# mratsim/constantine

Hardware: AMD Instinct MI355X
Metric: MSM points/sec, BLS12-381 G1, 2^20 random pairs; pipelined throughput, 2 MSMs in flight, inputs resident in HBM (higher is better)
Workload: dtype u32; 1 GPU; bls12_381_g1 MSM, 2^20 (scalar,point) pairs per GPU, inputs resident in HBM, 2 MSMs in flight (BASELINE.json configs[1]); pairs_per_gpu=1048576, total_pairs=1048576, ranks=1, scalar_bits=255, window_bits=16, windows=16, entries_per_lane=131, seed=1592590338

## Files before the change

constantine_amd/csrc/hip_backend.h:

```cpp
#pragma once
#include <hip/hip_runtime.h>

#include "generators.h"
#include "hip_errors.h"
#include "msm_pipeline.h"

namespace ctt {

#define HIP_CHECK(expr)                                                                              \
  do {                                                                                               \
    hipError_t e_ = (expr);                                                                          \
    if (e_ != hipSuccess)                                                                            \
      ::ctt::hip_failed(#expr, hipGetErrorString(e_), e_ == hipErrorOutOfMemory, __FILE__, __LINE__); \
  } while (0)

template <class Fr>
__global__ void k_fr_from_mont(const uint32_t* in, uint32_t* out, uint32_t n) {
  fr_from_mont_body<Fr>(in, out, n, blockIdx.x * blockDim.x + threadIdx.x);
}

static constexpr int ACCUM_BLOCK = 64;

static constexpr int EC_BLOCK = 64;

// ... 16 lines not shown
    const Affine<F> p = in[j];
    r.v.a.x = FD::from_sat(p.x);
    r.v.a.y = FD::from_sat(p.y);
    r.w[gather_flag_offset<FD>() / 4u] = p.is_inf() ? 1u : 0u;
#pragma unroll
    for (uint32_t i = 0; i < CH; i++) cv_lds[t * CH + (i ^ (t & (CH - 1u)))] = r.q[i];
  }
  __syncthreads();
  const uint32_t cnt = (n - j0 < (uint32_t)CONVERT_BLOCK ? n - j0 : (uint32_t)CONVERT_BLOCK) * CH;
  uint4* dst = reinterpret_cast<uint4*>((char*)out + (uint64_t)j0 * STRIDE);
  for (uint32_t i = t; i < cnt; i += CONVERT_BLOCK) {
    const uint32_t rec = i / CH, ch = i & (CH - 1u);
    dst[i] = cv_lds[rec * CH + (ch ^ (rec & (CH - 1u)))];
  }
}

#ifndef CTT_ACCUM_WAVES
#define CTT_ACCUM_WAVES 2
#endif
template <class F>
struct GatherLds {
  static constexpr uint32_t NCH = gather_chunks<F>();
  static_assert(F::UNSAT, "records in the converted layout only");
  uint4 (*stage)[ACCUM_BLOCK];
  __device__ void request(const char* rec) {
    asm volatile("s_waitcnt lgkmcnt(0)" ::: "memory");
#pragma unroll
    for (uint32_t j = 0; j < NCH; j++)
      __builtin_amdgcn_global_load_lds((const __attribute__((address_space(1))) void*)(rec + 16u * j),
                                       (__attribute__((address_space(3))) void*)&stage[j][0], 16, 0, 0);
  }
  __device__ void collect(Affine<F>& pt, bool& qinf) {
    asm volatile("s_waitcnt vmcnt(0)" ::: "memory");
    union {
      uint4 q[NCH];
      uint32_t w[NCH * 4u];
    } r;
#pragma unroll
    for (uint32_t j = 0; j < NCH; j++) r.q[j] = stage[j][threadIdx.x];
    __builtin_memcpy(&pt, r.w, sizeof(Affine<F>));
    qinf = r.w[gather_flag_offset<F>() / 4u] != 0u;
  }
};
template <class F, bool INTO = false>
__global__ void __launch_bounds__(ACCUM_BLOCK, (sizeof(XYZZ<F>) > 256 ? 1 : CTT_ACCUM_WAVES)) k_accum(AccumArgs<F> a) {
#if defined(CTT_G2_PHASE_NOPS) && CTT_G2_PHASE_NOPS > 0
  if constexpr (IsFp2<F>::value && F::UNSAT) {
#pragma unroll
    for (int i = 0; i < CTT_G2_PHASE_NOPS; i++) asm volatile("s_nop 0");
  }
#endif
  if constexpr (F::UNSAT && !IsFp2<F>::value) {
    __shared__ uint4 stage[GatherLds<F>::NCH][ACCUM_BLOCK];
    GatherLds<F> gq{stage};
    accum_body<F, GatherLds<F>, INTO>(a, blockIdx.y, blockIdx.x * blockDim.x + threadIdx.x, gq);
  } else {
    accum_body<F, INTO>(a, blockIdx.y, blockIdx.x * blockDim.x + threadIdx.x);
  }
}
template <class F>
__global__ void __launch_bounds__(EC_BLOCK) k_merge_tail(MergeArgs<F> a) {
  merge_tail_body<F>(a, blockIdx.y, blockIdx.x * blockDim.x + threadIdx.x);
}
template <class F>
__global__ void __launch_bounds__(EC_BLOCK) k_merge_step(MergeArgs<F> a, uint32_t d) {
  merge_step_body<F>(a, blockIdx.y, blockIdx.x * blockDim.x + threadIdx.x, d);
}
template <class F>
__global__ void __launch_bounds__(EC_BLOCK) k_merge_final(MergeArgs<F> a) {
  if (merge_chain_bound<F>(a) <= 1) return;
  merge_final_body<F>(a, blockIdx.y, blockIdx.x * blockDim.x + threadIdx.x);
}
template <class F>
__global__ void __launch_bounds__(EC_BLOCK) k_merge_tail_queue(MergeArgs<F> a) {
  uint32_t item = 0;
  const bool more = merge_tail_queue_body<F>(a, blockIdx.y, blockIdx.x * blockDim.x + threadIdx.x, &item);
  const uint64_t mask = __ballot(more);
  if (mask == 0) return;
  uint32_t base = 0;
  const uint32_t lane = threadIdx.x & 63u;
  if (lane == (uint32_t)(__ffsll((long long)mask) - 1)) base = atomicAdd(a.qcount, (uint32_t)__popcll(mask));
  base = __shfl(base, __ffsll((long long)mask) - 1, 64);
  if (more) a.queue[base + (uint32_t)__popcll(mask & ((1ull << lane) - 1ull))] = item;
}
template <class F>
__global__ void __launch_bounds__(EC_BLOCK) k_merge_queue(MergeArgs<F> a, uint32_t lmax) {
  merge_queue_body<F>(a, blockIdx.x * blockDim.x + threadIdx.x, lmax);
}
template <class F>
__global__ void __launch_bounds__(EC_BLOCK) k_pyr(PyrArgs<F> a, uint32_t ntasks) {
  const uint32_t t = blockIdx.x * blockDim.x + threadIdx.x;
  if (t < ntasks) pyr_body<F>(a, blockIdx.y, t);
}
// ... 180 lines not shown
    if (role == 0) {
      const XYZZ<F> x = *s1;
      *d1 = x;
      if (d2) *d2 = x;
    }
    return;
  }
  xyzz_add_quad<F>(s1, s2, d1, d2, role);
}
static constexpr int RED_BLOCK = 256;
template <class F>
__global__ void __launch_bounds__(RED_BLOCK) k_merge_finish(MergeArgs<F> a, uint32_t first_d) {
  merge_finish_body<F>(a, blockIdx.x, first_d, threadIdx.x, blockDim.x, []() { __syncthreads(); });
}
template <class F>
__global__ void __launch_bounds__(EC_BLOCK) k_merge_queue_quad(MergeArgs<F> a, uint32_t lmax) {
  const uint32_t lane = blockIdx.x * blockDim.x + threadIdx.x;
  const uint32_t qi = lane >> 2;
  const int role = (int)(lane & 3u);
  if (qi >= *a.qcount) return;
  const uint32_t slot = a.queue[qi];
  const uint32_t w = slot / a.G, s = slot - w * a.G;
  const uint32_t b = a.hkey[slot];
  const uint32_t* bs = a.bucket_start + (uint64_t)w * (a.B + 1);
  const uint32_t len = chain_last(bs, a.K, b) - s + 1;
  if (len > lmax) return;
  XYZZ<F> acc = a.heads[slot];
  for (uint32_t i = 1; i < len; i++) {
    const XYZZ<F> h = a.heads[slot + i];
    xyzz_add_quad_reg<F>(acc, h, role);
  }
  if (role == 0) a.buckets[(uint64_t)w * a.B + b] = acc;
}
template <class F>
__global__ void __launch_bounds__(RED_BLOCK) k_merge_long(MergeArgs<F> a, uint32_t lmax) {
  merge_long_body<F>(a, blockIdx.x, lmax, threadIdx.x, blockDim.x, []() { __syncthreads(); });
}
template <class F>
__global__ void __launch_bounds__(EC_BLOCK) k_merge_step_quad(MergeArgs<F> a, uint32_t d) {
  const uint32_t lane = blockIdx.x * blockDim.x + threadIdx.x;
  const uint32_t g = lane >> 2;
  if (!merge_step_active<F>(a, blockIdx.y, g, d)) return;
  XYZZ<F>* h = a.heads + (uint64_t)blockIdx.y * a.G + g;
  xyzz_add_quad<F>(h, h + d, h, (XYZZ<F>*)nullptr, (int)(lane & 3u));
}
template <class C>
__global__ void __launch_bounds__(EC_BLOCK) k_gen_points(uint64_t seed, uint64_t first, uint32_t n, Affine<typename C::F>* out) {
  Affine<typename C::F> G = generator<C>();
// ... 291 lines not shown
  }

  static dim3 grid1(uint32_t n, int block) { return dim3((n + block - 1) / block); }
  static dim3 grid2(uint32_t n, int block, uint32_t W) { return dim3((n + block - 1) / block, W); }

  template <class Fr>
  void launch_fr_from_mont(const uint32_t* in, uint32_t* out, uint32_t n) {
    hipLaunchKernelGGL(k_fr_from_mont<Fr>, grid1(n, 256), dim3(256), 0, front(), in, out, n);
    HIP_CHECK(hipGetLastError());
  }
  template <class F, class FD>
  void launch_convert(const Affine<F>* in, void* out, uint32_t n) {
    hipLaunchKernelGGL((k_convert_points<F, FD>), grid1(n, CONVERT_BLOCK), dim3(CONVERT_BLOCK),
                       (size_t)CONVERT_BLOCK * gather_stride<FD>(), front(), in, out, n);
    HIP_CHECK(hipGetLastError());
  }
  template <class F>
  void launch_table_next(const Affine<F>* prev, Affine<F>* next, uint32_t n, int c) {
    hipLaunchKernelGGL(k_table_next<F>, grid1(n, EC_BLOCK), dim3(EC_BLOCK), 0, stream, prev, next, n, c);
    HIP_CHECK(hipGetLastError());
  }
  void sync() { HIP_CHECK(hipStreamSynchronize(stream)); }
  void launch_digits_sort(const SortArgs& a);
  template <class F>
  void launch_accum(const AccumArgs<F>& a, uint32_t W, bool into = false) {
    if (into) launch_accum_into<F>(stream, a, W);
    else hipLaunchKernelGGL((k_accum<F, false>), grid2(a.G, ACCUM_BLOCK, W), dim3(ACCUM_BLOCK), 0, stream, a);
    HIP_CHECK(hipGetLastError());
  }
  template <class F>
  void launch_merge_tail(const MergeArgs<F>& a, uint32_t W) {
    hipLaunchKernelGGL(k_merge_tail<F>, grid2(a.G, EC_BLOCK, W), dim3(EC_BLOCK), 0, cur(), a);
    HIP_CHECK(hipGetLastError());
  }
  template <class F>
  void launch_merge_step(const MergeArgs<F>& a, uint32_t W, uint32_t d) {
    if ((uint64_t)a.G * W * 4u <= 1048576u) {
      hipLaunchKernelGGL(k_merge_step_quad<F>, grid2(a.G * 4u, EC_BLOCK, W), dim3(EC_BLOCK), 0, cur(), a, d);
      HIP_CHECK(hipGetLastError());
      return;
    }
    hipLaunchKernelGGL(k_merge_step<F>, grid2(a.G, EC_BLOCK, W), dim3(EC_BLOCK), 0, cur(), a, d);
    HIP_CHECK(hipGetLastError());
  }
  template <class F>
  void launch_merge_finish(const MergeArgs<F>& a, uint32_t W, uint32_t first_d) {
// ... 280 lines not shown
```

constantine_amd/csrc/msm_bodies.h:

```cpp
#pragma once
#include "ec.h"

namespace ctt {

static constexpr uint32_t DIGIT_NONE = 0xffffffffu;
static constexpr uint32_t KEY_NONE = 0xffffffffu;

struct Bls12381G1 { using F = Fp<BLS12_381_Fp>; using FD = FpU<BLS12_381_Fp_U>; using Fr = Fp<BLS12_381_Fr>; static constexpr int BITS = 255; static constexpr int ID = 0; static constexpr double ACC_NS = 0.142, RED_NS = 0.26; static constexpr int NARROW_PRIO_LOG2N = 19; static constexpr int WHOLE_TAIL_LOG2N = 0; };
struct Bls12381G2 { using F = Fp2<Fp<BLS12_381_Fp>>; using FD = Fp2<FpU<BLS12_381_Fp_U>>; using Fr = Fp<BLS12_381_Fr>; static constexpr int BITS = 255; static constexpr int ID = 1; static constexpr double ACC_NS = 0.467, RED_NS = 1.1; static constexpr int NARROW_PRIO_LOG2N = 0; static constexpr int WHOLE_TAIL_LOG2N = 0; };
struct Bn254G1 { using F = Fp<BN254_Fp>; using FD = FpU<BN254_Fp_U>; using Fr = Fp<BN254_Fr>; static constexpr int BITS = 254; static constexpr int ID = 2; static constexpr double ACC_NS = 0.0685, RED_NS = 0.12; static constexpr int NARROW_PRIO_LOG2N = 19; static constexpr int WHOLE_TAIL_LOG2N = 21; };
struct Bn254G2 { using F = Fp2<Fp<BN254_Fp>>; using FD = F; using Fr = Fp<BN254_Fr>; static constexpr int BITS = 254; static constexpr int ID = 3; static constexpr double ACC_NS = 0.5, RED_NS = 1.2; static constexpr int NARROW_PRIO_LOG2N = 0; static constexpr int WHOLE_TAIL_LOG2N = 0; };
struct PallasEc { using F = Fp<Pallas_Fp>; using FD = FpU<Pallas_Fp_U>; using Fr = Fp<Vesta_Fp>; static constexpr int BITS = 255; static constexpr int ID = 4; static constexpr double ACC_NS = 0.056, RED_NS = 0.10; static constexpr int NARROW_PRIO_LOG2N = 0; static constexpr int WHOLE_TAIL_LOG2N = 21; };
struct VestaEc { using F = Fp<Vesta_Fp>; using FD = FpU<Vesta_Fp_U>; using Fr = Fp<Pallas_Fp>; static constexpr int BITS = 255; static constexpr int ID = 5; static constexpr double ACC_NS = 0.056, RED_NS = 0.10; static constexpr int NARROW_PRIO_LOG2N = 0; static constexpr int WHOLE_TAIL_LOG2N = 21; };
struct Banderwagon { using F = Fp<Banderwagon_Fp>; using FD = F; using Fr = Fp<Banderwagon_Fr>; static constexpr int BITS = 253; static constexpr int ID = 6; static constexpr double ACC_NS = 0.12, RED_NS = 0.20; static constexpr int NARROW_PRIO_LOG2N = 0; static constexpr int WHOLE_TAIL_LOG2N = 0; };

CTT_HD uint32_t scalar_bits_at(const uint32_t* k, int pos, int nb) {
  int word = pos >> 5, sh = pos & 31;
  uint32_t lo = word < 8 ? k[word] >> sh : 0u;
  if (sh + nb > 32 && word + 1 < 8) lo |= k[word + 1] << (32 - sh);
  return lo & ((1u << nb) - 1u);
}

struct WinLayout {
  int cb, r;
// ... 109 lines not shown
CTT_HD void convert_point_body(const Affine<F>* in, void* out, uint32_t n, uint32_t j) {
  if (j >= n) return;
  Affine<F> p = in[j];
  Affine<FD> q;
  q.x = FD::from_sat(p.x);
  q.y = FD::from_sat(p.y);
  char* rec = (char*)out + (uint64_t)j * gather_stride<FD>();
  *(Affine<FD>*)rec = q;
  *(uint32_t*)(rec + gather_flag_offset<FD>()) = p.is_inf() ? 1u : 0u;
}

template <class F>
struct AccumArgs {
  const uint32_t* entries;
  const uint32_t* bucket_start;
  const void* points;
  uint32_t point_stride;
  XYZZ<F>* buckets;
  XYZZ<F>* heads;
  XYZZ<F>* tails;
  uint32_t* hkey;
  uint32_t* tkey;
  uint32_t N, B, K, G;
};

template <class F>
struct GatherDirect {
  const char* rec = nullptr;
  CTT_HD void request(const char* r) { rec = r; }
  CTT_HD void collect(Affine<F>& pt, bool& qinf) {
    pt = *(const Affine<F>*)rec;
    if constexpr (F::UNSAT) qinf = *(const uint32_t*)(rec + gather_flag_offset<F>()) != 0u; else qinf = pt.is_inf();
  }
};

struct BucketWalk {
  const uint32_t* bs;
  uint32_t B, b, bend, bend2;
  bool head0;
  CTT_HD void start(const uint32_t* bs_, uint32_t B_, uint32_t p0) {
    bs = bs_;
    B = B_;
    uint32_t lo = 0, hi = B;
    while (hi - lo > 1) {
      uint32_t mid = (lo + hi) >> 1;
      if (bs[mid] <= p0) lo = mid; else hi = mid;
    }
    b = lo;
    head0 = bs[b] < p0;
    bend = bs[b + 1];
    bend2 = bs[b + 2 <= B ? b + 2 : B];
  }
  CTT_HD void next(uint32_t pos) {
    b++;
    bend = bend2;
    while (bend == pos) {
      b++;
      bend = bs[b + 1];
    }
    bend2 = bs[b + 2 <= B ? b + 2 : B];
  }
};

template <class F, class G, bool INTO = false>
CTT_HD void accum_body_xyzz(const AccumArgs<F>& a, uint32_t w, uint32_t g, G& gq) {
  if (g >= a.G) return;
  const uint32_t* bs = a.bucket_start + (uint64_t)w * (a.B + 1);
  const uint64_t slot = (uint64_t)w * a.G + g;
  const uint32_t nw = bs[a.B];
  const uint64_t p0l = (uint64_t)g * a.K;
  uint32_t hk = KEY_NONE, tk = KEY_NONE;
  if (p0l >= nw) {
    a.hkey[slot] = hk;
    a.tkey[slot] = tk;
    return;
  }
  const uint32_t p0 = (uint32_t)p0l;
  const uint32_t p1 = (p0l + a.K < nw) ? p0 + a.K : nw;
  BucketWalk bw;
  bw.start(bs, a.B, p0);
  bool first_run = true;
  XYZZ<F> acc;
  bool empty = true;
  if constexpr (INTO) {
    if (!bw.head0) {
      acc = a.buckets[(uint64_t)w * a.B + bw.b];
      empty = acc.is_inf();
    }
  }
  const uint32_t* ent = a.entries + (uint64_t)w * a.N;
  auto record = [&](uint32_t e) {
    return (const char*)__builtin_assume_aligned((const char*)a.points + (uint64_t)(e & 0x7fffffffu) * a.point_stride, 16);
  };
  const uint32_t plast = p1 - 1;
  uint32_t e = ent[p0];
  uint32_t e1 = ent[p0 < plast ? p0 + 1 : plast];
  gq.request(record(e));
  for (uint32_t pos = p0; pos < p1; pos++) {
    Affine<F> pt;
    bool qinf;
    gq.collect(pt, qinf);
    if (pos == bw.bend) {
      if (empty) acc = XYZZ<F>::inf();
      if (first_run && bw.head0) {
        a.heads[slot] = acc;
        hk = bw.b;
      } else {
        a.buckets[(uint64_t)w * a.B + bw.b] = acc;
      }
      first_run = false;
      empty = true;
      bw.next(pos);
      if constexpr (INTO) {
        acc = a.buckets[(uint64_t)w * a.B + bw.b];
        empty = acc.is_inf();
      }
    }
    gq.request(record(e1));
    const uint32_t e2 = ent[pos + 2 < p1 ? pos + 2 : plast];
    if (!qinf) xyzz_madd_flag<F, SignMask>(acc, empty, pt.x, pt.y, SignMask(e));
    e = e1;
    e1 = e2;
  }
  if (empty) acc = XYZZ<F>::inf();
  const uint32_t b = bw.b;
  const bool started_before = first_run && bw.head0;
  const bool ends_after = bw.bend > p1;
  if (started_before) {
    a.heads[slot] = acc;
    hk = b;
  } else if (ends_after) {
    a.tails[slot] = acc;
    tk = b;
  } else {
    a.buckets[(uint64_t)w * a.B + b] = acc;
  }
  a.hkey[slot] = hk;
  a.tkey[slot] = tk;
}

template <class F, class Z, bool INTO = false>
CTT_HD void accum_body_z(const AccumArgs<F>& a, uint32_t w, uint32_t g, Z& z) {
  if (g >= a.G) return;
  const uint32_t* bs = a.bucket_start + (uint64_t)w * (a.B + 1);
  const uint64_t slot = (uint64_t)w * a.G + g;
// ... 82 lines not shown
    accum_body_z<F, ZInRegs<F>, INTO>(a, w, g, z);
  } else {
    accum_body_xyzz<F, G, INTO>(a, w, g, gq);
  }
}
template <class F, bool INTO = false>
CTT_HD void accum_body(const AccumArgs<F>& a, uint32_t w, uint32_t g) {
  GatherDirect<F> gq;
  accum_body<F, GatherDirect<F>, INTO>(a, w, g, gq);
}

template <class F>
struct MergeArgs {
  const uint32_t* bucket_start;
  XYZZ<F>* buckets;
  XYZZ<F>* heads;
  const XYZZ<F>* tails;
  const uint32_t* hkey;
  const uint32_t* tkey;
  const uint32_t* maxcount;
  uint32_t B, K, G;
  uint32_t* queue = nullptr;
  uint32_t* qcount = nullptr;
};

template <class F>
CTT_HD uint32_t merge_chain_bound(const MergeArgs<F>& a) {
  const uint32_t mc = *a.maxcount;
  return mc ? (mc - 1) / a.K + 1 : 0;
}

template <class F>
CTT_HD void merge_tail_body(const MergeArgs<F>& a, uint32_t w, uint32_t g) {
  if (g + 1 >= a.G) return;
  const uint64_t slot = (uint64_t)w * a.G + g;
  const uint32_t b = a.tkey[slot];
  if (b == KEY_NONE) return;
  const bool final_ = merge_chain_bound<F>(a) <= 1;
  XYZZ<F> h = a.heads[slot + 1];
  XYZZ<F> t = a.tails[slot];
  XYZZ<F> r = xyzz_add_inl<F>(h, t);
  if (final_) a.buckets[(uint64_t)w * a.B + b] = r; else a.heads[slot + 1] = r;
}

template <class F>
CTT_HD bool merge_step_active(const MergeArgs<F>& a, uint32_t w, uint32_t g, uint32_t d) {
  if (g >= a.G) return false;
  const uint32_t mc = *a.maxcount;
  if (mc == 0 || d >= (mc - 1) / a.K + 1) return false;
  const uint64_t slot = (uint64_t)w * a.G + g;
  const uint32_t b = a.hkey[slot];
  if (b == KEY_NONE) return false;
  const uint32_t* bs = a.bucket_start + (uint64_t)w * (a.B + 1);
  const uint32_t s = bs[b] / a.K + 1;
  const uint32_t e = (bs[b + 1] - 1) / a.K;
  const uint32_t rel = g - s;
  return (rel % (2 * d)) == 0 && g + d <= e;
}
template <class F>
CTT_HD void merge_step_body(const MergeArgs<F>& a, uint32_t w, uint32_t g, uint32_t d) {
  if (!merge_step_active<F>(a, w, g, d)) return;
  const uint64_t slot = (uint64_t)w * a.G + g;
  XYZZ<F> x = a.heads[slot];
  XYZZ<F> y = a.heads[slot + d];
  a.heads[slot] = xyzz_add_inl<F>(x, y);
}

template <class F>
CTT_HD void merge_final_body(const MergeArgs<F>& a, uint32_t w, uint32_t g) {
  if (g >= a.G) return;
  const uint64_t slot = (uint64_t)w * a.G + g;
  const uint32_t b = a.hkey[slot];
  if (b == KEY_NONE) return;
  const uint32_t* bs = a.bucket_start + (uint64_t)w * (a.B + 1);
  if (g != bs[b] / a.K + 1) return;
  a.buckets[(uint64_t)w * a.B + b] = a.heads[slot];
}

template <class F, class Sync>
CTT_HD void merge_finish_body(const MergeArgs<F>& a, uint32_t w, uint32_t first_d, uint32_t lane, uint32_t nlanes, Sync&& sync) {
  const uint32_t chain = merge_chain_bound<F>(a);
  for (uint32_t d = first_d; d < chain; d <<= 1) {
    for (uint32_t g = lane; g < a.G; g += nlanes) merge_step_body<F>(a, w, g, d);
    sync();
  }
}

CTT_HD uint32_t chain_first(const uint32_t* bs, uint32_t K, uint32_t b) { return bs[b] / K + 1; }
CTT_HD uint32_t chain_last(const uint32_t* bs, uint32_t K, uint32_t b) { return (bs[b + 1] - 1) / K; }

CTT_HD uint32_t merge_queue_capacity(uint32_t W, uint32_t G) { return W * (G / 2u + 1u); }

template <class F>
CTT_HD bool merge_tail_queue_body(const MergeArgs<F>& a, uint32_t w, uint32_t g, uint32_t* item) {
  if (g + 1 >= a.G) return false;
  const uint64_t slot = (uint64_t)w * a.G + g;
  const uint32_t b = a.tkey[slot];
  if (b == KEY_NONE) return false;
  const uint32_t* bs = a.bucket_start + (uint64_t)w * (a.B + 1);
  const XYZZ<F> h = a.heads[slot + 1], t = a.tails[slot];
  const XYZZ<F> r = xyzz_add_inl<F>(h, t);
  const bool more = chain_last(bs, a.K, b) > g + 1;
  if (more) {
    a.heads[slot + 1] = r;
    *item = (uint32_t)(slot + 1);
  } else {
    a.buckets[(uint64_t)w * a.B + b] = r;
  }
  return more;
}

template <class F>
CTT_HD void merge_queue_body(const MergeArgs<F>& a, uint32_t qi, uint32_t lmax) {
  if (qi >= *a.qcount) return;
  const uint32_t slot = a.queue[qi];
  const uint32_t w = slot / a.G, s = slot - w * a.G;
  const uint32_t b = a.hkey[slot];
  const uint32_t* bs = a.bucket_start + (uint64_t)w * (a.B + 1);
  const uint32_t len = chain_last(bs, a.K, b) - s + 1;
  if (len > lmax) return;
  XYZZ<F> r = a.heads[slot];
  for (uint32_t i = 1; i < len; i++) {
    const XYZZ<F> h = a.heads[slot + i];
    r = xyzz_add_inl<F>(r, h);
  }
  a.buckets[(uint64_t)w * a.B + b] = r;
}

template <class F, class Sync>
CTT_HD void merge_long_body(const MergeArgs<F>& a, uint32_t w, uint32_t lmax, uint32_t lane, uint32_t nlanes, Sync&& sync) {
  const uint32_t chain = merge_chain_bound<F>(a);
  if (chain <= lmax) return;
  const uint32_t* bs = a.bucket_start + (uint64_t)w * (a.B + 1);
  auto is_long = [&](uint32_t b) { return chain_last(bs, a.K, b) - chain_first(bs, a.K, b) + 1 > lmax; };
  for (uint32_t d = 1; d < chain; d <<= 1) {
    for (uint32_t g = lane; g < a.G; g += nlanes) {
      if (!merge_step_active<F>(a, w, g, d)) continue;
      const uint64_t slot = (uint64_t)w * a.G + g;
      if (!is_long(a.hkey[slot])) continue;
      const XYZZ<F> x = a.heads[slot], y = a.heads[slot + d];
      a.heads[slot] = xyzz_add_inl<F>(x, y);
    }
    sync();
  }
  for (uint32_t g = lane; g < a.G; g += nlanes) {
    const uint64_t slot = (uint64_t)w * a.G + g;
    const uint32_t b = a.hkey[slot];
    if (b == KEY_NONE || g != chain_first(bs, a.K, b) || !is_long(b)) continue;
    a.buckets[(uint64_t)w * a.B + b] = a.heads[slot];
  }
}

template <class F>
struct PyrArgs {
  const XYZZ<F>* buckets;
  XYZZ<F>* pyr;
  XYZZ<F>* q;
  XYZZ<F>* out;
  uint32_t B;
  int c;
  int p;
  uint32_t out_stride;
};

template <class F>
CTT_HD const XYZZ<F>* pyr_level(const PyrArgs<F>& a, uint32_t w, int l) {
  if (l == 0) return a.buckets + (uint64_t)w * a.B;
  return a.pyr + (uint64_t)w * a.B + (a.B - (a.B >> (l - 1)));
}

CTT_HD uint32_t pyr_pass_tasks(uint32_t B, int c, int p) {
// ... 389 lines not shown
```

constantine_amd/csrc/msm_engine.hip:

```cpp
#include <memory>
#include <mutex>
#include <atomic>
#include <system_error>
#include <thread>
#include <vector>

#if defined(__linux__)
#include <pthread.h>
#include <sched.h>
#endif

#include "hip_backend.h"

using namespace ctt;

#include <stdarg.h>
namespace ctt {
ErrorState& error_state() {
  static thread_local ErrorState st;
  return st;
}
void set_last_error(int code, const char* fmt, ...) {
  ErrorState& st = error_state();
  st.code = code;
// ... 137 lines not shown
  const uint32_t* src = in + (uint64_t)blockIdx.x * len;
  uint32_t* dst = out + (uint64_t)blockIdx.x * (len + 1);
  if (tid == 0) carry_s = 0;
  __syncthreads();
  for (uint32_t b0 = 0; b0 < len; b0 += 1024u) {
    const uint32_t b = b0 + tid;
    const uint32_t v = b < len ? src[b] : 0u;
    uint32_t x = v;
#pragma unroll
    for (uint32_t off = 1; off < 64; off <<= 1) {
      const uint32_t y = __shfl_up(x, off, 64);
      if (lane >= off) x += y;
    }
    if (lane == 63) wsum[wv] = x;
    __syncthreads();
    uint32_t base = carry_s;
    for (uint32_t k = 0; k < wv; k++) base += wsum[k];
    if (b < len) dst[b] = base + x - v;
    __syncthreads();
    if (tid == 1023) carry_s = base + x;
    __syncthreads();
  }
  if (tid == 0) dst[len] = carry_s;
}

template <bool MERGED>
__global__ void __launch_bounds__(1024) k_part_scatter(SortArgs a, uint32_t w0, uint32_t nw) {
  extern __shared__ uint32_t lds[];
  const uint32_t ncnt = MERGED ? a.NG : nw * a.NG;
  const uint32_t wstep = MERGED ? 0u : a.NG;
  uint32_t* cur = lds;
  const uint32_t set0 = MERGED ? 0u : w0;
  const uint32_t blk = part_slice_of_block(a, blockIdx.x, gridDim.x);
  const uint32_t* off = a.cntA + (uint64_t)blk * (a.W * a.NG) + (uint64_t)set0 * a.NG;
  for (uint32_t i = threadIdx.x; i < ncnt; i += blockDim.x) {
    const uint32_t w = i / a.NG, g = i - w * a.NG;
    cur[i] = off[i] + a.gbase[(uint64_t)(set0 + w) * (a.NG + 1) + g];
  }
  __syncthreads();
  const uint32_t j0 = blk * a.slice;
  const uint32_t j1 = (j0 + a.slice < a.n) ? j0 + a.slice : a.n;
  const uint32_t sh = a.jbits + 1u;
  for (uint32_t jb = j0; jb < j1; jb += PS_NS * blockDim.x) {
    uint32_t k[PS_NS][8];
    load_scalars<PS_NS>(a, jb, j1, k);
    for_each_digit<PS_NS>(k, w0, nw, a.lay, [&](uint32_t w, const uint32_t (&d)[PS_NS]) {
// ... 338 lines not shown
  }
  hipLaunchKernelGGL(k_part_scan_blocks, dim3((ncol + SCAN_CX - 1) / SCAN_CX), dim3(1024), 0, front(), a.cntA, a.gtot, ncol, a.nblk);
  HIP_CHECK(hipGetLastError());
  hipLaunchKernelGGL(k_scan_u32, dim3(a.W), dim3(1024), 0, front(), (const uint32_t*)a.gtot, a.gbase, a.NG);
  HIP_CHECK(hipGetLastError());
  if (a.staged && a.NG <= 1024u && (a.NG & (a.NG - 1u)) == 0u) {
    const size_t rec = a.merged ? 8 : 4;
    const size_t lds_bytes = ((size_t)3 * a.NG + 16) * 4 + (size_t)PS_NS * 1024 * (2 + rec);
    if (a.merged) hipLaunchKernelGGL(k_part_scatter_staged<true>, dim3(a.nblk), dim3(1024), lds_bytes, front(), a);
    else hipLaunchKernelGGL(k_part_scatter_staged<false>, dim3(a.nblk), dim3(1024), lds_bytes, front(), a);
    HIP_CHECK(hipGetLastError());
  } else {
    for (uint32_t w0 = 0; w0 < a.Wd; w0 += wb) {
      const uint32_t nw = (w0 + wb <= a.Wd) ? wb : a.Wd - w0;
      if (a.merged) hipLaunchKernelGGL(k_part_scatter<true>, dim3(a.nblk), dim3(1024), (size_t)a.NG * 4, front(), a, w0, nw);
      else hipLaunchKernelGGL(k_part_scatter<false>, dim3(a.nblk), dim3(1024), (size_t)nw * a.NG * 4, front(), a, w0, nw);
      HIP_CHECK(hipGetLastError());
    }
  }
  const uint32_t Bg = a.B / a.NG;
  const size_t lds = ((size_t)2 * Bg + 1 + a.cap + a.big) * 4;
  if (a.merged) hipLaunchKernelGGL(k_group_sort<true>, dim3(a.W * a.NG), dim3(1024), lds, front(), a);
  else hipLaunchKernelGGL(k_group_sort<false>, dim3(a.W * a.NG), dim3(1024), lds, front(), a);
  HIP_CHECK(hipGetLastError());
}

static constexpr int NUM_CURVES = 7;

static const CurveOps* curve_ops(int id) {
  switch (id) {
    case 0: return ctt_ops_bls12_381_g1();
    case 1: return ctt_ops_bls12_381_g2();
    case 2: return ctt_ops_bn254_snarks_g1();
    case 3: return ctt_ops_bn254_snarks_g2();
    case 4: return ctt_ops_pallas();
    case 5: return ctt_ops_vesta();
    case 6: return ctt_ops_banderwagon();
  }
  return nullptr;
}

static bool out_kind_ok(int curve, int out_kind) {
  return out_kind == OUT_AFF || out_kind == OUT_PRJ || (out_kind == OUT_JAC && curve != Banderwagon::ID);
}
static bool is_weierstrass(int curve) { return curve != Banderwagon::ID; }

// ... 975 lines not shown
```

constantine_amd/csrc/msm_pipeline.h:

```cpp
#pragma once
#include <stdio.h>
#include <stdlib.h>
#include <string.h>

#include <atomic>
#include <functional>
#include <system_error>
#include <thread>
#include <type_traits>
#include <vector>

#include "host_fp64.h"
#include "msm_bodies.h"

namespace ctt {

struct OutOfDeviceMemory { size_t bytes; };

struct MsmPlan {
  uint32_t n;
  int c, W;
  uint32_t B;
  uint32_t S;
  uint32_t slice;
  uint32_t NG;
  uint32_t gshift;
  uint32_t gshift_narrow;
  WinLayout lay;
  uint32_t jbits;
  uint32_t cap, big;
  uint32_t K;
  uint32_t G;
// ... 336 lines not shown
      if (tab) bk.free(tab);
      if (lvl[0]) bk.free(lvl[0]);
      *c_out = 0;
      return nullptr;
    }
    const Affine<F>* cur = d_points_in;
    for (int w = 0; w < Wd; w++) {
      if (w > 0) {
        Affine<F>* nxt = lvl[w & 1];
        bk.template launch_table_next<F>(cur, nxt, n, lay.width((uint32_t)w - 1));
        cur = nxt;
      }
      if constexpr (kConvert) bk.template launch_convert<F, FD>(cur, tab + (size_t)w * n * stride, n);
      else bk.d2d_async(tab + (size_t)w * n * stride, cur, (size_t)n * sizeof(Affine<F>));
    }
    bk.sync();
    bk.free(lvl[0]);
    bk.free(lvl[1]);
    return tab;
  }

  struct Staged {
    uint32_t* d_bstart;
    uint32_t* d_maxcount;
    XYZZ<FD>* d_buckets;
    XYZZ<FD>* d_heads;
    XYZZ<FD>* d_tails;
    uint32_t* d_hkey;
    uint32_t* d_tkey;
  };
  void reserve_stage1(int sl, const MsmPlan& p, bool coef_is_fr) {
    const size_t W = p.W, n = p.nent;
    if (coef_is_fr) need(scal, (size_t)p.n * 32);
    need(part, W * n * (p.merged ? 8 : 4));
    need(counts, (size_t)p.S * W * p.NG * 4);
    need(totals, W * p.NG * 4);
    need(gbase, W * (p.NG + 1) * 4);
    need(bstartS[sl], W * (p.B + 1) * 4);
    need(entries, W * n * 4);
    need(maxcountS[sl], 256);
    need(heads, W * p.G * sizeof(XYZZ<FD>));
    need(tails, W * p.G * sizeof(XYZZ<FD>));
    need(hkey, W * p.G * 4);
    need(tkey, W * p.G * 4);
    if (p.merge_lmax > 0) need(mqueue, (size_t)merge_queue_capacity(p.W, p.G) * 4);
  }
  Staged accumulate_pairs(int sl, const MsmPlan& p, const uint32_t* d_coefs, bool coef_is_fr, const Affine<F>* d_points_in,
                          const void* d_prepared, void* d_converted, XYZZ<FD>* d_buckets, bool into = false,
                          const std::function<void()>* points_arrive = nullptr, bool front_side = false) {
    const uint32_t n = p.n, W = p.W, B = p.B;
    if (front_side) bk.front_begin();
    bk.stage_begin(sl, ST_DIGITS);
    const uint32_t* d_scalars = d_coefs;
    if (coef_is_fr) {
      uint32_t* t = (uint32_t*)need(scal, (size_t)n * 32);
      bk.template launch_fr_from_mont<typename C::Fr>(d_coefs, t, n);
      d_scalars = t;
    }
    const void* d_points;
    uint32_t point_stride;
    const bool convert_late = points_arrive != nullptr;
// ... 6 lines not shown
      }
      point_stride = gather_stride<FD>();
    } else {
      d_points = d_prepared ? d_prepared : (const void*)d_points_in;
      point_stride = (uint32_t)sizeof(Affine<F>);
    }
    bk.stage_end(sl, ST_DIGITS);

    bk.stage_begin(sl, ST_SORT);
    SortArgs sa;
    sa.scalars = d_scalars;
    sa.n = n; sa.c = p.c; sa.lay = p.lay; sa.W = W; sa.B = B;
    sa.Wd = (uint32_t)p.Wd; sa.merged = p.merged; sa.nent = p.nent; sa.id_stride = p.id_stride;
    sa.NG = p.NG; sa.gshift = p.gshift; sa.gshift_narrow = p.gshift_narrow; sa.slice = p.slice; sa.nblk = p.S;
    sa.jbits = p.jbits;
    sa.cap = p.cap; sa.big = p.big;
    sa.xcd_map = opt.sort_xcd ? 1u : 0u;
    sa.staged = (opt.sort_staged >= 2 || (opt.sort_staged == 1 && p.NG >= 256u)) ? 1u : 0u;
    sa.part = (uint32_t*)need(part, (size_t)W * p.nent * (p.merged ? 8 : 4));
    sa.cntA = (uint32_t*)need(counts, (size_t)p.S * W * p.NG * 4);
    sa.gtot = (uint32_t*)need(totals, (size_t)W * p.NG * 4);
    sa.gbase = (uint32_t*)need(gbase, (size_t)W * (p.NG + 1) * 4);
    Staged st;
    st.d_bstart = (uint32_t*)need(bstartS[sl], (size_t)W * (B + 1) * 4);
    uint32_t* d_entries = (uint32_t*)need(entries, (size_t)W * p.nent * 4);
    st.d_maxcount = (uint32_t*)need(maxcountS[sl], 256);
    sa.bstart = st.d_bstart; sa.entries = d_entries; sa.maxcount = st.d_maxcount;
    sa.zero_base = into ? nullptr : (void*)d_buckets;
    sa.zero_bytes = into ? 0u : (uint32_t)sizeof(XYZZ<FD>);
    bk.launch_digits_sort(sa);
    if (convert_late) {
      (*points_arrive)();
      if constexpr (kConvert) {
        if (!d_prepared) bk.template launch_convert<F, FD>(d_points_in, d_converted, n);
      }
    }
    bk.stage_end(sl, ST_SORT);
    if (front_side) bk.front_end();

    const uint64_t accum_waves = (uint64_t)W * ((p.G + 63u) / 64u);
    const bool whole_tail = C::WHOLE_TAIL_LOG2N > 0 && p.n >= (1u << C::WHOLE_TAIL_LOG2N);
    if (!bk.partitioned() && (whole_tail || accum_waves + tail_min_free_waves() > (uint64_t)opt.lanes / 64u)) bk.tail_wait();
    bk.wide_wait();
    bk.stage_begin(sl, ST_ACCUM);
    st.d_buckets = d_buckets;
    st.d_heads = (XYZZ<FD>*)need(heads, (size_t)W * p.G * sizeof(XYZZ<FD>));
    st.d_tails = (XYZZ<FD>*)need(tails, (size_t)W * p.G * sizeof(XYZZ<FD>));
    st.d_hkey = (uint32_t*)need(hkey, (size_t)W * p.G * 4);
    st.d_tkey = (uint32_t*)need(tkey, (size_t)W * p.G * 4);
    AccumArgs<FD> aa{d_entries, st.d_bstart, d_points, point_stride, d_buckets, st.d_heads, st.d_tails, st.d_hkey, st.d_tkey, p.nent, B, p.K, p.G};
    bk.template launch_accum<FD>(aa, W, into);
    bk.accum_mark(front_side);
    bk.stage_end(sl, ST_ACCUM);
    return st;
  }

  void merge_buckets(int sl, const MsmPlan& p, const Staged& st) {
    bk.stage_begin(sl, ST_MERGE);
    MergeArgs<FD> ma{st.d_bstart, st.d_buckets, st.d_heads, st.d_tails, st.d_hkey, st.d_tkey, st.d_maxcount, p.B, p.K, p.G};
    if (p.merge_lmax > 0) {
      ma.queue = (uint32_t*)need(mqueue, (size_t)merge_queue_capacity(p.W, p.G) * 4);
      ma.qcount = st.d_maxcount + 2;
      bk.template launch_merge_tail_queue<FD>(ma, p.W);
      bk.template launch_merge_queue<FD>(ma, p.W, p.merge_lmax, opt.merge_queue_quad != 2);
      bk.template launch_merge_long<FD>(ma, p.W, p.merge_lmax);
    } else {
      bk.template launch_merge_tail<FD>(ma, p.W);
      uint32_t d = 1;
      for (int i = 0; i < p.merge_steps && d < p.G; i++, d <<= 1) bk.template launch_merge_step<FD>(ma, p.W, d);
      bk.template launch_merge_finish<FD>(ma, p.W, d);
    }
    bk.stage_end(sl, ST_MERGE);
  }

  void reduce_buckets(int sl, const MsmPlan& p, XYZZ<FD>* d_buckets) {
    Slot& S = slots[sl];
    const uint32_t W = p.W, B = p.B;
    const bool forked_early = bk.tail_forked();
    if (!forked_early) bk.tail_wait();
    bk.stage_begin(sl, ST_REDUCE);
    XYZZ<FD>* d_pyr = (XYZZ<FD>*)need(rA[0], (size_t)W * B * sizeof(XYZZ<FD>));
    XYZZ<FD>* d_q = (XYZZ<FD>*)need(rA[1], (size_t)W * (B / 2 + 1) * sizeof(XYZZ<FD>));
// ... 407 lines not shown
```

Before: 382.6 million points/s.

## Balance accumulation lanes by bucket-slot prefix and pair first two adds

Adds a per-window slot-prefix kernel that counts, for each bucket, the additions it needs (m-1 for buckets with two or more entries). Lanes then split work by equal numbers of additions instead of equal numbers of entries, using a binary search over the prefix. The accumulator loop now fills the empty accumulator with two points at once: it loads the first point, then adds the second, so the first point of each bucket run no longer costs a full mixed add. The gather stage is double-buffered in LDS so the next two records can be prefetched. In exchange this adds an extra kernel launch, binary searches per lane, more LDS use, and merge-chain bounds that are now computed per window.

Measured after the change: 368.2 million points/s. -3.8%, worse.

```diff
diff --git a/constantine_amd/csrc/hip_backend.h b/constantine_amd/csrc/hip_backend.h
--- a/constantine_amd/csrc/hip_backend.h
+++ b/constantine_amd/csrc/hip_backend.h
@@ -62,22 +62,34 @@
 struct GatherLds {
   static constexpr uint32_t NCH = gather_chunks<F>();
   static_assert(F::UNSAT, "records in the converted layout only");
-  uint4 (*stage)[ACCUM_BLOCK];
-  __device__ void request(const char* rec) {
-    asm volatile("s_waitcnt lgkmcnt(0)" ::: "memory");
+  uint4 (*stage)[NCH][ACCUM_BLOCK];
+  template <int S>
+  __device__ void issue(const char* rec) {
 #pragma unroll
     for (uint32_t j = 0; j < NCH; j++)
       __builtin_amdgcn_global_load_lds((const __attribute__((address_space(1))) void*)(rec + 16u * j),
-                                       (__attribute__((address_space(3))) void*)&stage[j][0], 16, 0, 0);
-  }
-  __device__ void collect(Affine<F>& pt, bool& qinf) {
+                                       (__attribute__((address_space(3))) void*)&stage[S][j][0], 16, 0, 0);
+  }
+  __device__ void request(uint32_t s, const char* rec) {
+    asm volatile("s_waitcnt lgkmcnt(0)" ::: "memory");
+    if (s == 0) issue<0>(rec); else issue<1>(rec);
+  }
+  __device__ void refill(uint32_t cur, const char* ra, bool two, const char* rb) {
+    asm volatile("s_waitcnt lgkmcnt(0)" ::: "memory");
+    if (cur == 0 || two) issue<0>(cur == 0 ? ra : rb);
+    if (cur != 0 || two) issue<1>(cur != 0 ? ra : rb);
+  }
+  __device__ void collect(uint32_t s, Affine<F>& pt, bool& qinf) {
     asm volatile("s_waitcnt vmcnt(0)" ::: "memory");
+    collect_second(s, pt, qinf);
+  }
+  __device__ void collect_second(uint32_t s, Affine<F>& pt, bool& qinf) {
     union {
       uint4 q[NCH];
       uint32_t w[NCH * 4u];
     } r;
 #pragma unroll
-    for (uint32_t j = 0; j < NCH; j++) r.q[j] = stage[j][threadIdx.x];
+    for (uint32_t j = 0; j < NCH; j++) r.q[j] = stage[s][j][threadIdx.x];
     __builtin_memcpy(&pt, r.w, sizeof(Affine<F>));
     qinf = r.w[gather_flag_offset<F>() / 4u] != 0u;
   }
@@ -91,7 +103,7 @@
   }
 #endif
   if constexpr (F::UNSAT && !IsFp2<F>::value) {
-    __shared__ uint4 stage[GatherLds<F>::NCH][ACCUM_BLOCK];
+    __shared__ uint4 stage[2][GatherLds<F>::NCH][ACCUM_BLOCK];
     GatherLds<F> gq{stage};
     accum_body<F, GatherLds<F>, INTO>(a, blockIdx.y, blockIdx.x * blockDim.x + threadIdx.x, gq);
   } else {
@@ -108,7 +120,7 @@
 }
 template <class F>
 __global__ void __launch_bounds__(EC_BLOCK) k_merge_final(MergeArgs<F> a) {
-  if (merge_chain_bound<F>(a) <= 1) return;
+  if (merge_chain_bound<F>(a, blockIdx.y) <= 1) return;
   merge_final_body<F>(a, blockIdx.y, blockIdx.x * blockDim.x + threadIdx.x);
 }
 template <class F>
@@ -335,8 +347,7 @@
   const uint32_t slot = a.queue[qi];
   const uint32_t w = slot / a.G, s = slot - w * a.G;
   const uint32_t b = a.hkey[slot];
-  const uint32_t* bs = a.bucket_start + (uint64_t)w * (a.B + 1);
-  const uint32_t len = chain_last(bs, a.K, b) - s + 1;
+  const uint32_t len = merge_ranges<F>(a, w).chain_last(b) - s + 1;
   if (len > lmax) return;
   XYZZ<F> acc = a.heads[slot];
   for (uint32_t i = 1; i < len; i++) {
@@ -674,6 +685,7 @@
   }
   void sync() { HIP_CHECK(hipStreamSynchronize(stream)); }
   void launch_digits_sort(const SortArgs& a);
+  void launch_slot_prefix(const uint32_t* bstart, uint32_t* slot_prefix, uint32_t W, uint32_t B);
   template <class F>
   void launch_accum(const AccumArgs<F>& a, uint32_t W, bool into = false) {
     if (into) launch_accum_into<F>(stream, a, W);
diff --git a/constantine_amd/csrc/msm_bodies.h b/constantine_amd/csrc/msm_bodies.h
--- a/constantine_amd/csrc/msm_bodies.h
+++ b/constantine_amd/csrc/msm_bodies.h
@@ -155,15 +155,54 @@
   uint32_t* hkey;
   uint32_t* tkey;
   uint32_t N, B, K, G;
-};
+  const uint32_t* slot_prefix = nullptr;
+};
+
+static constexpr uint32_t LANE_SLOTS_MIN = 4;
+struct LaneRanges {
+  const uint32_t* bs;
+  const uint32_t* sp;
+  uint32_t B, K;
+  CTT_HD LaneRanges(const uint32_t* bucket_start, const uint32_t* slot_prefix, uint32_t w, uint32_t B_, uint32_t K_, uint32_t G)
+      : bs(bucket_start + (uint64_t)w * (B_ + 1)), sp(slot_prefix ? slot_prefix + (uint64_t)w * (B_ + 1) : nullptr), B(B_), K(K_) {
+    if (sp) {
+      K = sp[B] / G + 1u;
+      if (K < LANE_SLOTS_MIN) K = LANE_SLOTS_MIN;
+    }
+  }
+  CTT_HD uint32_t begin(uint32_t g) const {
+    const uint64_t T = (uint64_t)g * K;
+    const uint32_t nw = bs[B];
+    if (!sp) return T < nw ? (uint32_t)T : nw;
+    if (T == 0) return 0;
+    if (T > sp[B]) return nw;
+    uint32_t lo = 0, hi = B;
+    while (hi - lo > 1) {
+      const uint32_t mid = (lo + hi) >> 1;
+      if (sp[mid] < T) lo = mid; else hi = mid;
+    }
+    const uint32_t s = bs[lo], m = bs[lo + 1] - s;
+    return s + ((uint32_t)T - sp[lo]) + (m >= 2 ? 1u : 0u);
+  }
+  CTT_HD uint32_t chain_first(uint32_t b) const { return (sp ? sp : bs)[b] / K + 1; }
+  CTT_HD uint32_t chain_last(uint32_t b) const { return ((sp ? sp : bs)[b + 1] - 1) / K; }
+  CTT_HD uint32_t chain_bound(uint32_t mc) const { return mc ? (mc - 1) / K + 1 : 0; }
+};
+CTT_HD uint32_t bucket_slots(uint32_t m) { return m >= 2 ? m - 1 : m; }
 
 template <class F>
 struct GatherDirect {
-  const char* rec = nullptr;
-  CTT_HD void request(const char* r) { rec = r; }
-  CTT_HD void collect(Affine<F>& pt, bool& qinf) {
-    pt = *(const Affine<F>*)rec;
-    if constexpr (F::UNSAT) qinf = *(const uint32_t*)(rec + gather_flag_offset<F>()) != 0u; else qinf = pt.is_inf();
+  const char* rec[2] = {nullptr, nullptr};
+  CTT_HD void request(uint32_t s, const char* r) { rec[s] = r; }
+  CTT_HD void refill(uint32_t cur, const char* ra, bool two, const char* rb) {
+    rec[cur] = ra;
+    if (two) rec[cur ^ 1u] = rb;
+  }
+  CTT_HD void collect_second(uint32_t s, Affine<F>& pt, bool& qinf) { collect(s, pt, qinf); }
+  CTT_HD void collect(uint32_t s, Affine<F>& pt, bool& qinf) {
+    const char* r = rec[s];
+    pt = *(const Affine<F>*)r;
+    if constexpr (F::UNSAT) qinf = *(const uint32_t*)(r + gather_flag_offset<F>()) != 0u; else qinf = pt.is_inf();
   }
 };
 
@@ -198,18 +237,18 @@
 template <class F, class G, bool INTO = false>
 CTT_HD void accum_body_xyzz(const AccumArgs<F>& a, uint32_t w, uint32_t g, G& gq) {
   if (g >= a.G) return;
-  const uint32_t* bs = a.bucket_start + (uint64_t)w * (a.B + 1);
+  const LaneRanges lr(a.bucket_start, a.slot_prefix, w, a.B, a.K, a.G);
+  const uint32_t* bs = lr.bs;
   const uint64_t slot = (uint64_t)w * a.G + g;
   const uint32_t nw = bs[a.B];
-  const uint64_t p0l = (uint64_t)g * a.K;
+  const uint32_t p0 = lr.begin(g);
   uint32_t hk = KEY_NONE, tk = KEY_NONE;
-  if (p0l >= nw) {
+  if (p0 >= nw) {
     a.hkey[slot] = hk;
     a.tkey[slot] = tk;
     return;
   }
-  const uint32_t p0 = (uint32_t)p0l;
-  const uint32_t p1 = (p0l + a.K < nw) ? p0 + a.K : nw;
+  const uint32_t p1 = lr.begin(g + 1);
   BucketWalk bw;
   bw.start(bs, a.B, p0);
   bool first_run = true;
@@ -226,13 +265,16 @@
     return (const char*)__builtin_assume_aligned((const char*)a.points + (uint64_t)(e & 0x7fffffffu) * a.point_stride, 16);
   };
   const uint32_t plast = p1 - 1;
-  uint32_t e = ent[p0];
-  uint32_t e1 = ent[p0 < plast ? p0 + 1 : plast];
-  gq.request(record(e));
-  for (uint32_t pos = p0; pos < p1; pos++) {
+  auto word = [&](uint32_t p) { return ent[p < plast ? p : plast]; };
+  uint32_t e0 = word(p0), e1 = word(p0 + 1), e2 = word(p0 + 2), e3 = word(p0 + 3);
+  gq.request(0, record(e0));
+  gq.request(1, record(e1));
+  uint32_t cur = 0;
+  uint32_t pos = p0;
+  while (pos < p1) {
     Affine<F> pt;
     bool qinf;
-    gq.collect(pt, qinf);
+    gq.collect(cur, pt, qinf);
     if (pos == bw.bend) {
       if (empty) acc = XYZZ<F>::inf();
       if (first_run && bw.head0) {
@@ -249,11 +291,35 @@
         empty = acc.is_inf();
       }
     }
-    gq.request(record(e1));
-    const uint32_t e2 = ent[pos + 2 < p1 ? pos + 2 : plast];
-    if (!qinf) xyzz_madd_flag<F, SignMask>(acc, empty, pt.x, pt.y, SignMask(e));
-    e = e1;
-    e1 = e2;
+    uint32_t e = e0;
+    bool add = !qinf, two = false;
+    if (empty && add) {
+      bool start = true;
+      xyzz_madd_flag<F, SignMask>(acc, start, pt.x, pt.y, SignMask(e0));
+      empty = false;
+      add = false;
+      if (pos + 1 < p1 && pos + 1 != bw.bend) {
+        gq.collect_second(cur ^ 1u, pt, qinf);
+        e = e1;
+        add = !qinf;
+        two = true;
+      }
+    }
+    gq.refill(cur, record(e2), two, record(e3));
+    if (two) {
+      pos += 2;
+      e0 = e2;
+      e1 = e3;
+      e2 = word(pos + 2);
+    } else {
+      pos += 1;
+      cur ^= 1u;
+      e0 = e1;
+      e1 = e2;
+      e2 = e3;
+    }
+    e3 = word(pos + 3);
+    if (add) xyzz_madd_flag<F, SignMask>(acc, empty, pt.x, pt.y, SignMask(e));
   }
   if (empty) acc = XYZZ<F>::inf();
   const uint32_t b = bw.b;
@@ -382,11 +448,17 @@
   uint32_t B, K, G;
   uint32_t* queue = nullptr;
   uint32_t* qcount = nullptr;
-};
-
+  const uint32_t* slot_prefix = nullptr;
+};
+template <class F>
+CTT_HD LaneRanges merge_ranges(const MergeArgs<F>& a, uint32_t w) { return LaneRanges(a.bucket_start, a.slot_prefix, w, a.B, a.K, a.G); }
+
+template <class F>
+CTT_HD uint32_t merge_chain_bound(const MergeArgs<F>& a, uint32_t w) { return merge_ranges<F>(a, w).chain_bound(*a.maxcount); }
 template <class F>
 CTT_HD uint32_t merge_chain_bound(const MergeArgs<F>& a) {
   const uint32_t mc = *a.maxcount;
+  if (a.slot_prefix) return mc;
   return mc ? (mc - 1) / a.K + 1 : 0;
 }
 
@@ -396,7 +468,7 @@
   const uint64_t slot = (uint64_t)w * a.G + g;
   const uint32_t b = a.tkey[slot];
   if (b == KEY_NONE) return;
-  const bool final_ = merge_chain_bound<F>(a) <= 1;
+  const bool final_ = merge_chain_bound<F>(a, w) <= 1;
   XYZZ<F> h = a.heads[slot + 1];
   XYZZ<F> t = a.tails[slot];
   XYZZ<F> r = xyzz_add_inl<F>(h, t);
@@ -406,14 +478,13 @@
 template <class F>
 CTT_HD bool merge_step_active(const MergeArgs<F>& a, uint32_t w, uint32_t g, uint32_t d) {
   if (g >= a.G) return false;
-  const uint32_t mc = *a.maxcount;
-  if (mc == 0 || d >= (mc - 1) / a.K + 1) return false;
+  const LaneRanges lr = merge_ranges<F>(a, w);
+  if (d >= lr.chain_bound(*a.maxcount)) return false;
   const uint64_t slot = (uint64_t)w * a.G + g;
   const uint32_t b = a.hkey[slot];
   if (b == KEY_NONE) return false;
-  const uint32_t* bs = a.bucket_start + (uint64_t)w * (a.B + 1);
-  const uint32_t s = bs[b] / a.K + 1;
-  const uint32_t e = (bs[b + 1] - 1) / a.K;
+  const uint32_t s = lr.chain_first(b);
+  const uint32_t e = lr.chain_last(b);
   const uint32_t rel = g - s;
   return (rel % (2 * d)) == 0 && g + d <= e;
 }
@@ -432,22 +503,19 @@
   const uint64_t slot = (uint64_t)w * a.G + g;
   const uint32_t b = a.hkey[slot];
   if (b == KEY_NONE) return;
-  const uint32_t* bs = a.bucket_start + (uint64_t)w * (a.B + 1);
-  if (g != bs[b] / a.K + 1) return;
+  if (g != merge_ranges<F>(a, w).chain_first(b)) return;
   a.buckets[(uint64_t)w * a.B + b] = a.heads[slot];
 }
 
 template <class F, class Sync>
 CTT_HD void merge_finish_body(const MergeArgs<F>& a, uint32_t w, uint32_t first_d, uint32_t lane, uint32_t nlanes, Sync&& sync) {
-  const uint32_t chain = merge_chain_bound<F>(a);
+  const uint32_t chain = merge_chain_bound<F>(a, w);
   for (uint32_t d = first_d; d < chain; d <<= 1) {
     for (uint32_t g = lane; g < a.G; g += nlanes) merge_step_body<F>(a, w, g, d);
     sync();
   }
 }
 
-CTT_HD uint32_t chain_first(const uint32_t* bs, uint32_t K, uint32_t b) { return bs[b] / K + 1; }
-CTT_HD uint32_t chain_last(const uint32_t* bs, uint32_t K, uint32_t b) { return (bs[b + 1] - 1) / K; }
 
 CTT_HD uint32_t merge_queue_capacity(uint32_t W, uint32_t G) { return W * (G / 2u + 1u); }
 
@@ -457,10 +525,9 @@
   const uint64_t slot = (uint64_t)w * a.G + g;
   const uint32_t b = a.tkey[slot];
   if (b == KEY_NONE) return false;
-  const uint32_t* bs = a.bucket_start + (uint64_t)w * (a.B + 1);
   const XYZZ<F> h = a.heads[slot + 1], t = a.tails[slot];
   const XYZZ<F> r = xyzz_add_inl<F>(h, t);
-  const bool more = chain_last(bs, a.K, b) > g + 1;
+  const bool more = merge_ranges<F>(a, w).chain_last(b) > g + 1;
   if (more) {
     a.heads[slot + 1] = r;
     *item = (uint32_t)(slot + 1);
@@ -476,8 +543,7 @@
   const uint32_t slot = a.queue[qi];
   const uint32_t w = slot / a.G, s = slot - w * a.G;
   const uint32_t b = a.hkey[slot];
-  const uint32_t* bs = a.bucket_start + (uint64_t)w * (a.B + 1);
-  const uint32_t len = chain_last(bs, a.K, b) - s + 1;
+  const uint32_t len = merge_ranges<F>(a, w).chain_last(b) - s + 1;
   if (len > lmax) return;
   XYZZ<F> r = a.heads[slot];
   for (uint32_t i = 1; i < len; i++) {
@@ -489,10 +555,10 @@
 
 template <class F, class Sync>
 CTT_HD void merge_long_body(const MergeArgs<F>& a, uint32_t w, uint32_t lmax, uint32_t lane, uint32_t nlanes, Sync&& sync) {
-  const uint32_t chain = merge_chain_bound<F>(a);
+  const uint32_t chain = merge_chain_bound<F>(a, w);
   if (chain <= lmax) return;
-  const uint32_t* bs = a.bucket_start + (uint64_t)w * (a.B + 1);
-  auto is_long = [&](uint32_t b) { return chain_last(bs, a.K, b) - chain_first(bs, a.K, b) + 1 > lmax; };
+  const LaneRanges lr = merge_ranges<F>(a, w);
+  auto is_long = [&](uint32_t b) { return lr.chain_last(b) - lr.chain_first(b) + 1 > lmax; };
   for (uint32_t d = 1; d < chain; d <<= 1) {
     for (uint32_t g = lane; g < a.G; g += nlanes) {
       if (!merge_step_active<F>(a, w, g, d)) continue;
@@ -506,7 +572,7 @@
   for (uint32_t g = lane; g < a.G; g += nlanes) {
     const uint64_t slot = (uint64_t)w * a.G + g;
     const uint32_t b = a.hkey[slot];
-    if (b == KEY_NONE || g != chain_first(bs, a.K, b) || !is_long(b)) continue;
+    if (b == KEY_NONE || g != lr.chain_first(b) || !is_long(b)) continue;
     a.buckets[(uint64_t)w * a.B + b] = a.heads[slot];
   }
 }
diff --git a/constantine_amd/csrc/msm_engine.hip b/constantine_amd/csrc/msm_engine.hip
--- a/constantine_amd/csrc/msm_engine.hip
+++ b/constantine_amd/csrc/msm_engine.hip
@@ -183,6 +183,37 @@
     __syncthreads();
   }
   if (tid == 0) dst[len] = carry_s;
+}
+
+__global__ void __launch_bounds__(1024) k_slot_prefix(const uint32_t* __restrict__ bstart, uint32_t* __restrict__ sp, uint32_t B) {
+  __shared__ uint32_t wsum[16];
+  const uint32_t tid = threadIdx.x, lane = tid & 63u, wv = tid >> 6;
+  const uint32_t* bs = bstart + (uint64_t)blockIdx.x * (B + 1);
+  uint32_t* dst = sp + (uint64_t)blockIdx.x * (B + 1);
+  const uint32_t seg = (B + 15u) / 16u;
+  const uint64_t s0l = (uint64_t)wv * seg;
+  const uint32_t s0 = s0l < B ? (uint32_t)s0l : B, s1 = s0l + seg < B ? (uint32_t)(s0l + seg) : B;
+  uint32_t v = 0;
+  for (uint32_t b = s0 + lane; b < s1; b += 64u) v += bucket_slots(bs[b + 1] - bs[b]);
+#pragma unroll
+  for (uint32_t off = 32; off >= 1; off >>= 1) v += __shfl_xor(v, off, 64);
+  if (lane == 0) wsum[wv] = v;
+  __syncthreads();
+  uint32_t base = 0;
+  for (uint32_t k = 0; k < wv; k++) base += wsum[k];
+  for (uint32_t b0 = s0; b0 < s1; b0 += 64u) {
+    const uint32_t b = b0 + lane;
+    const uint32_t c = b < s1 ? bucket_slots(bs[b + 1] - bs[b]) : 0u;
+    uint32_t x = c;
+#pragma unroll
+    for (uint32_t off = 1; off < 64; off <<= 1) {
+      const uint32_t y = __shfl_up(x, off, 64);
+      if (lane >= off) x += y;
+    }
+    if (b < s1) dst[b] = base + x - c;
+    base += __shfl(x, 63, 64);
+  }
+  if (tid == 1023) dst[B] = base;
 }
 
 template <bool MERGED>
@@ -567,6 +598,11 @@
   const size_t lds = ((size_t)2 * Bg + 1 + a.cap + a.big) * 4;
   if (a.merged) hipLaunchKernelGGL(k_group_sort<true>, dim3(a.W * a.NG), dim3(1024), lds, front(), a);
   else hipLaunchKernelGGL(k_group_sort<false>, dim3(a.W * a.NG), dim3(1024), lds, front(), a);
+  HIP_CHECK(hipGetLastError());
+}
+
+void HipBackend::launch_slot_prefix(const uint32_t* bstart, uint32_t* slot_prefix, uint32_t W, uint32_t B) {
+  hipLaunchKernelGGL(k_slot_prefix, dim3(W), dim3(1024), 0, front(), bstart, slot_prefix, B);
   HIP_CHECK(hipGetLastError());
 }
 
diff --git a/constantine_amd/csrc/msm_pipeline.h b/constantine_amd/csrc/msm_pipeline.h
--- a/constantine_amd/csrc/msm_pipeline.h
+++ b/constantine_amd/csrc/msm_pipeline.h
@@ -8,6 +8,7 @@
 #include <system_error>
 #include <thread>
 #include <type_traits>
+#include <utility>
 #include <vector>
 
 #include "host_fp64.h"
@@ -390,6 +391,7 @@
 
   struct Staged {
     uint32_t* d_bstart;
+    uint32_t* d_slot_prefix;
     uint32_t* d_maxcount;
     XYZZ<FD>* d_buckets;
     XYZZ<FD>* d_heads;
@@ -397,6 +399,12 @@
     uint32_t* d_hkey;
     uint32_t* d_tkey;
   };
+  template <class B, class = void>
+  struct HasSlotPrefix : std::false_type {};
+  template <class B>
+  struct HasSlotPrefix<B, std::void_t<decltype(std::declval<B&>().launch_slot_prefix((const uint32_t*)nullptr, (uint32_t*)nullptr, 0u, 0u))>> : std::true_type {};
+  static constexpr bool kSlotRanges = HasSlotPrefix<BK>::value && !(IsFp2<FD>::value && FD::UNSAT);
+  static size_t bstart_bytes(const MsmPlan& p) { return (size_t)p.W * (p.B + 1) * 4 * (kSlotRanges ? 2 : 1); }
   void reserve_stage1(int sl, const MsmPlan& p, bool coef_is_fr) {
     const size_t W = p.W, n = p.nent;
     if (coef_is_fr) need(scal, (size_t)p.n * 32);
@@ -404,7 +412,7 @@
     need(counts, (size_t)p.S * W * p.NG * 4);
     need(totals, W * p.NG * 4);
     need(gbase, W * (p.NG + 1) * 4);
-    need(bstartS[sl], W * (p.B + 1) * 4);
+    need(bstartS[sl], bstart_bytes(p));
     need(entries, W * n * 4);
     need(maxcountS[sl], 256);
     need(heads, W * p.G * sizeof(XYZZ<FD>));
@@ -457,13 +465,15 @@
     sa.gtot = (uint32_t*)need(totals, (size_t)W * p.NG * 4);
     sa.gbase = (uint32_t*)need(gbase, (size_t)W * (p.NG + 1) * 4);
     Staged st;
-    st.d_bstart = (uint32_t*)need(bstartS[sl], (size_t)W * (B + 1) * 4);
+    st.d_bstart = (uint32_t*)need(bstartS[sl], bstart_bytes(p));
+    st.d_slot_prefix = kSlotRanges ? st.d_bstart + (size_t)W * (B + 1) : nullptr;
     uint32_t* d_entries = (uint32_t*)need(entries, (size_t)W * p.nent * 4);
     st.d_maxcount = (uint32_t*)need(maxcountS[sl], 256);
     sa.bstart = st.d_bstart; sa.entries = d_entries; sa.maxcount = st.d_maxcount;
     sa.zero_base = into ? nullptr : (void*)d_buckets;
     sa.zero_bytes = into ? 0u : (uint32_t)sizeof(XYZZ<FD>);
     bk.launch_digits_sort(sa);
+    if constexpr (kSlotRanges) bk.launch_slot_prefix(st.d_bstart, st.d_slot_prefix, W, B);
     if (convert_late) {
       (*points_arrive)();
       if constexpr (kConvert) {
@@ -484,6 +494,7 @@
     st.d_hkey = (uint32_t*)need(hkey, (size_t)W * p.G * 4);
     st.d_tkey = (uint32_t*)need(tkey, (size_t)W * p.G * 4);
     AccumArgs<FD> aa{d_entries, st.d_bstart, d_points, point_stride, d_buckets, st.d_heads, st.d_tails, st.d_hkey, st.d_tkey, p.nent, B, p.K, p.G};
+    aa.slot_prefix = st.d_slot_prefix;
     bk.template launch_accum<FD>(aa, W, into);
     bk.accum_mark(front_side);
     bk.stage_end(sl, ST_ACCUM);
@@ -493,6 +504,7 @@
   void merge_buckets(int sl, const MsmPlan& p, const Staged& st) {
     bk.stage_begin(sl, ST_MERGE);
     MergeArgs<FD> ma{st.d_bstart, st.d_buckets, st.d_heads, st.d_tails, st.d_hkey, st.d_tkey, st.d_maxcount, p.B, p.K, p.G};
+    ma.slot_prefix = st.d_slot_prefix;
     if (p.merge_lmax > 0) {
       ma.queue = (uint32_t*)need(mqueue, (size_t)merge_queue_capacity(p.W, p.G) * 4);
       ma.qcount = st.d_maxcount + 2;
```
